# seqsense/pcgol

Hardware: AMD Instinct MI355X
Metric: Mpoints/sec ICP iter (corr+reduce) + kNN queries/sec, 1M-pt cloud (higher is better)
Workload: dtype f32

## Files before the change

pcgol_amd/csrc/icp.hip:

```cpp
#include <string.h>

#include <array>
#include <chrono>
#include <condition_variable>
#include <mutex>
#include <string>
#include <thread>

#include <vector>

#include "knn_grid.h"
#include "knn_xwalk.h"
#include "strict_terms.h"

namespace pcgx {

constexpr int kIcpBlock = kKnnBlock;

__device__ __forceinline__ double wave_sum_f64(double v) {
#pragma unroll
  for (int o = 32; o > 0; o >>= 1) v += __shfl_down(v, o);
  return v;
}

// ... 145 lines not shown
      return;
    }
  }
  uint32_t *queue = s_stack + (size_t)(tv.depth > 1 ? tv.depth - 1 : 1) * kIcpBlock +
                    (threadIdx.x >> 6) * (kWalkQueueBytesPerWave / 4);
  float *top = reinterpret_cast<float *>(s_stack + (size_t)(tv.depth > 1 ? tv.depth - 1 : 1) * kIcpBlock +
                                         (kIcpBlock / 64) * (kWalkQueueBytesPerWave / 4));
  load_top_levels(tv, top);
  uint32_t chunk_begin, chunk_end;
  block_chunk_range(nt, blockIdx.x, gridDim.x, chunk_begin, chunk_end);
  if (threadIdx.x == 0) s_next_chunk = chunk_begin;
  __syncthreads();
  float m[16];
#pragma unroll
  for (int i = 0; i < 16; i++) m[i] = state->trans[i];
  const bool project = state->iter > 0;
  auto load_query = [&](int64_t i, float &x, float &y, float &z, float &ub, uint32_t &pred) {
    const float x0 = tx[i], y0 = ty[i], z0 = tz[i];
    float4 pm = make_float4(0.0f, 0.0f, 0.0f, -1.0f);
    pred = 0u;
    if (project) {
      pred = first_leaf[i] & 0x7fffffffu;
      if (!kMinDist) pm = match[i];
    }
    x = x0; y = y0; z = z0;
    if (project) mat4_transform(m, x0, y0, z0, x, y, z);
    const float dx = pm.x - x, dy = pm.y - y, dz = pm.z - z;
    const float dm = (dx * dx + dy * dy) + dz * dz;
    ub = dm + (pm.w >= 0.0f ? 0.0f : __builtin_inff());
  };
  auto emit = [&](int64_t i, const float4 &bp, float best_d) {
    const float4 rec = make_float4(bp.x, bp.y, bp.z, __float_as_int(bp.w) >= 0 ? best_d : -1.0f);
    match[i] = rec;
    if (match_caller) match_caller[orig_of[i]] = rec;
    if (kPlane) match_id[i] = __float_as_uint(bp.w);
    if (match_cert) match_cert[i] = (cert_by_id && __float_as_int(bp.w) >= 0) ? cert_by_id[__float_as_uint(bp.w)] : 0.0f;
  };
  if (kGrid) {
    const int64_t r_begin = (int64_t)chunk_begin * 64;
    __syncthreads();
    if (threadIdx.x == 0) {
      walk_count[slot] = 0;
      s_next_chunk = 0;
    }
    __syncthreads();
    walk_queries<kMinDist>(
        tv, s_stack + threadIdx.x, kIcpBlock, queue, top, (int64_t)left, &s_next_chunk, (left + 63u) / 64u, 0,
        kp.max_dist_sq, kp.min_dist_sq,
        [&](int64_t j, float &x, float &y, float &z, float &ub, uint32_t &pred) {
          load_query(r_begin + walk_list[r_begin + j], x, y, z, ub, pred);
          pred &= 0x7fffffffu;
        },
        [&](int64_t j, const float4 &bp, float best_d) { emit(r_begin + walk_list[r_begin + j], bp, best_d); },
        [&](int64_t j, uint32_t leaf) { first_leaf[r_begin + walk_list[r_begin + j]] = kSums ? (leaf | 0x80000000u) : leaf; });
    if (!kSums) {
      __syncthreads();
      strict_tile_sums();
      return;
    }
    __threadfence_block();
    __syncthreads();
    reduce_block_range<kPlane, true>(s_stack, tx, ty, tz, nt, chunk_begin, chunk_end, project, m, match, match_id,
                                     normals, kp, block_partials, first_leaf, grid_part);
    return;
  } else {
    walk_queries<kMinDist>(
        tv, s_stack + threadIdx.x, kIcpBlock, queue, top, nt, &s_next_chunk, chunk_end, (int64_t)chunk_begin * 64,
// ... 58 lines not shown
      if (test_force_walk && i % test_force_walk == 0) kept = false;
      if (kTrace && match_cert != nullptr && grid.cert != nullptr && pm.w >= 0.0f && dm < match_cert[i] && dm < kp.max_dist_sq)
        atomicAdd(&trace[36], 1ull);
    }
    float4 best = make_float4(0.0f, 0.0f, 0.0f, __int_as_float(-1));
    float best_d = kp.max_dist_sq;
    GridTrace tr;
    GridVerdict v = GRID_FOUND;
    if (kept) {
      best = make_float4(pm.x, pm.y, pm.z, __int_as_float(0));
      best_d = dm;
    } else {
      v = grid_nearest(grid, x, y, z, kp.max_dist_sq, ub, best, best_d, kTrace ? &tr : nullptr);
      if (test_force_walk && project && i % test_force_walk == 0) v = GRID_WALK;
    }
    if (use_cert && !kept)
      match_cert[i] = (v == GRID_FOUND && __float_as_int(best.w) >= 0) ? grid.cert[__float_as_uint(best.w)] : 0.0f;
    if (kTrace) {
      if (v == GRID_WALK) atomicAdd(&trace[0], 1ull);
      atomicAdd(&trace[1], (unsigned long long)tr.points);
      atomicAdd(&trace[2], (unsigned long long)tr.words);
      if (tr.wave_slots) atomicAdd(&trace[3], (unsigned long long)tr.wave_slots);
      atomicAdd(&trace[4 + (tr.rounds4 < 0 ? 0 : min(tr.rounds4 + 1, 15))], 1ull);
      atomicAdd(&trace[20 + (tr.rounds9 < 0 ? 0 : min(tr.rounds9 + 1, 15))], 1ull);
    } else if (v == GRID_WALK) {
      uint32_t begin;
      const uint32_t slot = slot_of_query(nt, i, n_corr_blocks, begin);
      const int64_t r_begin = (int64_t)begin * 64;
      walk_list[r_begin + atomicAdd(&walk_count[slot], 1u)] = (uint32_t)(i - r_begin);
      first_leaf[i] = kSums ? 0x80000000u : 0u;
      if (!walk_follows) const_cast<IcpState *>(state)->done = 2;
      if (!kSums && match_caller) {
        const bool seen = __float_as_int(best.w) >= 0;
        match_caller[orig_of[i]] = make_float4(best.x, best.y, best.z, seen ? best_d : -1.0f);
      }
    } else {
      const bool found = __float_as_int(best.w) >= 0;
      const float4 bp = make_float4(best.x, best.y, best.z, found ? best_d : -1.0f);
      if (kept) reinterpret_cast<float *>(&match[i])[3] = bp.w;
      else match[i] = bp;
      if (!kSums && match_caller && !(kept && caller_has_pairs)) match_caller[orig_of[i]] = bp;
      if (kPlane && !kept) match_id[i] = __float_as_uint(best.w);
      if (found && kSums) {
        if (kPlane) accumulate_plane_terms(acc, x, y, z, bp, normals[kept ? match_id[i] : __float_as_uint(best.w)]);
        else accumulate_terms(acc, x, y, z, bp, kp);
      }
    }
  }
  if (kTrace || !kSums) return;
  constexpr int kSub = kPlane ? 8 : 16, kRun = kIcpGridBlock / kSub;
  static_assert(NS * kSub <= kIcpGridBlock, "one lane per (component, run)");
#pragma unroll
  for (int k = 0; k < NS; k++) s_terms[k][threadIdx.x] = (float)acc[k];
  __syncthreads();
  if (threadIdx.x < NS * kSub) {
    const int k = threadIdx.x / kSub, j = threadIdx.x % kSub;
    double v = 0.0;
    for (int u = 0; u < kRun; u++) v += (double)s_terms[k][u * kSub + j];
#pragma unroll
    for (int o = kSub / 2; o > 0; o >>= 1) v += __shfl_down(v, o, kSub);
    if (j == 0) block_partials[((int64_t)n_corr_blocks + tile) * NS + k] = v;
  }
}

template <bool kMinDist, bool kPlane, bool kSums = true>
__global__ __launch_bounds__(kIcpBlock) void icp_corr_xkernel(
    XTreeView xv, const float *__restrict__ tx, const float *__restrict__ ty, const float *__restrict__ tz,
    int64_t nt, const IcpState *__restrict__ state, IcpKernelParams kp, float4 *__restrict__ match,
    double *__restrict__ block_partials, uint32_t *__restrict__ match_id, const float4 *__restrict__ normals,
    int64_t guard) {
  extern __shared__ uint32_t s_stack[];
  if (state->done) return;
  uint32_t chunk_begin, chunk_end;
  block_chunk_range(nt, blockIdx.x, gridDim.x, chunk_begin, chunk_end);
// ... 152 lines not shown

using namespace pcgx;

struct pcgx_icp_session {
  const pcgx_kdtree *base = nullptr;
  bool patched = false;
  int64_t nt = 0;
  float *d_xyz = nullptr;
  IcpState *d_state = nullptr;
  double *d_partials = nullptr;
  uint32_t *d_pos_of = nullptr;
  uint32_t *d_orig_of = nullptr;
  float4 *d_match_caller = nullptr;
  bool caller_order_fresh = false;
  bool tile_sums_fresh = false;
  int strict = 0;
  bool strict_explicit = false;
  pcgx::StrictBuffers *strict_buf = nullptr;
  float *d_terms = nullptr;
  unsigned long long *d_valid = nullptr;
  int64_t nt_pad = 0;
  float4 *d_match = nullptr;
  float *d_match_cert = nullptr;
  uint32_t *d_first_leaf = nullptr;
  uint32_t *d_walk_list = nullptr;
  uint32_t *d_walk_count = nullptr;
  double *d_sums = nullptr;
  bool own_sums = false;
  double *d_xchg = nullptr;
  int32_t steps_sharded = 0;
  int32_t host_iter = 0;
  bool spec_walk = true;
  bool spec_pending = false;
  hipStream_t spec_stream = nullptr;
  hipStream_t used[4] = {nullptr, nullptr, nullptr, nullptr};
  int n_used = 0;
  void touch(hipStream_t st) {
    for (int k = 0; k < n_used && k < 4; k++)
      if (used[k] == st) return;
    if (n_used > 0) (void)hipStreamSynchronize(used[0]);
    if (n_used < 4) used[n_used] = st;
    n_used++;
  }
  bool shard_failed = false;
  bool ring_fit_open = false;
  bool general_ready = true;
  bool small = false;
  int32_t *d_small_perm = nullptr;
  void *d_small_sync = nullptr;
  bool plane = false;
  uint32_t *d_match_id = nullptr;
  float4 *d_normals = nullptr;
  int n_sums() const { return plane ? (int)P_COUNT : (int)S_COUNT; }
  int grid = 1;
  IcpKernelParams kp;
  int32_t max_iteration = 20;
};

static pcgx_status settle(pcgx_icp_session *s, hipStream_t st);
static int icp_knob(const char *name, int def, int lo, int hi);

static IcpKernelParams make_kernel_params(const pcgx_icp_params *p) {
  IcpKernelParams kp;
  memset(&kp, 0, sizeof kp);
  kp.max_dist_sq = p->max_dist * p->max_dist;
  kp.min_dist_sq = p->min_dist_sq;
// ... 11 lines not shown
  if (blocks > cap) blocks = cap;
  if (blocks >= 8) blocks &= ~(int64_t)7;
  if (blocks < 1) blocks = 1;
  return (int)blocks;
}

__global__ void icp_reset_kernel(IcpState *__restrict__ state) {
  if (threadIdx.x != 0 || blockIdx.x != 0) return;
  IcpState h;
  memset(&h, 0, sizeof h);
  const Mat4 id = mat4_translate(0.0f, 0.0f, 0.0f);
  for (int i = 0; i < 16; i++) h.trans[i] = id.m[i];
  *state = h;
}

static pcgx_status general_prepare(pcgx_icp_session *s, hipStream_t st) {
  if (s->general_ready) return PCGX_OK;
  const size_t n1 = (size_t)(s->nt ? s->nt : 1);
  PCGX_HIP_TRY(hipMemsetAsync(s->d_match, 0xFF, n1 * sizeof(float4), st));
  PCGX_HIP_TRY(hipMemsetAsync(s->d_match_cert, 0, n1 * sizeof(float), st));
  PCGX_HIP_TRY(hipMemsetAsync(s->d_first_leaf, 0, n1 * sizeof(uint32_t), st));
  PCGX_HIP_TRY(hipMemsetAsync(s->d_walk_count, 0, (size_t)s->grid * sizeof(uint32_t), st));
  s->general_ready = true;
  return PCGX_OK;
}

static pcgx_status reset_state(pcgx_icp_session *s, hipStream_t st) {
  hipLaunchKernelGGL(icp_reset_kernel, dim3(1), dim3(64), 0, st, s->d_state);
  PCGX_HIP_TRY(hipGetLastError());
  s->host_iter = 0;
  if (s->spec_pending) {
    s->spec_pending = false;
    if (s->d_walk_count) PCGX_HIP_TRY(hipMemsetAsync(s->d_walk_count, 0, (size_t)s->grid * sizeof(uint32_t), st));
  }
  if (s->shard_failed || s->steps_sharded > 0) {
    PCGX_TRY(strict_reset(s->strict_buf, st));
    s->shard_failed = false;
    s->steps_sharded = 0;
  }
  return PCGX_OK;
}

extern "C" pcgx_status pcgx_icp_session_reset(pcgx_icp_session *s, void *stream) {
  PCGX_API_LOCK();
  if (!s) return fail(PCGX_E_INVALID, "pcgx_icp_session_reset: NULL session");
  s->touch(pick_stream(stream));
  return reset_state(s, pick_stream(stream));
}

extern "C" pcgx_status pcgx_icp_session_set_pose(pcgx_icp_session *s, const float trans16[16],
                                                 int32_t iter, void *stream) {
  PCGX_API_LOCK();
  if (!s || !trans16 || iter < 0) return fail(PCGX_E_INVALID, "pcgx_icp_session_set_pose: bad argument");
  hipStream_t st = pick_stream(stream);
  s->touch(st);
  PCGX_TRY(settle(s, st));
  IcpState h;
  memset(&h, 0, sizeof h);
  memcpy(h.trans, trans16, sizeof h.trans);
  h.iter = iter;
  s->host_iter = 0;
  PCGX_HIP_TRY(hipMemcpyAsync(s->d_state, &h, sizeof h, hipMemcpyHostToDevice, st));
  PCGX_HIP_TRY(hipStreamSynchronize(st));
  return PCGX_OK;
}

// ... 244 lines not shown
  }
  return def;
}

static pcgx_status enqueue_corr_patched(pcgx_icp_session *s, hipStream_t st) {
  XTreeView xv;
  PCGX_TRY(xtree_view(s->base, &xv, st));
  const size_t lds = (size_t)(xv.depth > 1 ? xv.depth : 2) * kIcpBlock * sizeof(uint32_t);
  const int64_t guard = 4 * s->base->n + 8;
  const float *x = s->d_xyz, *y = s->d_xyz + s->nt, *z = s->d_xyz + 2 * s->nt;
  ProfScope prof(PCGX_PROF_ICP_WALK, st);
  if (s->plane)
    hipLaunchKernelGGL((icp_corr_xkernel<false, true>), dim3(s->grid), dim3(kIcpBlock), lds, st, xv, x, y, z, s->nt,
                       s->d_state, s->kp, s->d_match, s->d_partials, s->d_match_id, (const float4 *)s->d_normals, guard);
  else if (s->kp.min_dist_sq > 0.0f && s->strict)
    hipLaunchKernelGGL((icp_corr_xkernel<true, false, false>), dim3(s->grid), dim3(kIcpBlock), lds, st, xv, x, y, z, s->nt,
                       s->d_state, s->kp, s->d_match, s->d_partials, (uint32_t *)nullptr, (const float4 *)nullptr, guard);
  else if (s->kp.min_dist_sq > 0.0f)
    hipLaunchKernelGGL((icp_corr_xkernel<true, false>), dim3(s->grid), dim3(kIcpBlock), lds, st, xv, x, y, z, s->nt,
                       s->d_state, s->kp, s->d_match, s->d_partials, (uint32_t *)nullptr, (const float4 *)nullptr, guard);
  else if (s->strict)
    hipLaunchKernelGGL((icp_corr_xkernel<false, false, false>), dim3(s->grid), dim3(kIcpBlock), lds, st, xv, x, y, z, s->nt,
                       s->d_state, s->kp, s->d_match, s->d_partials, (uint32_t *)nullptr, (const float4 *)nullptr, guard);
  else
    hipLaunchKernelGGL((icp_corr_xkernel<false, false>), dim3(s->grid), dim3(kIcpBlock), lds, st, xv, x, y, z, s->nt,
                       s->d_state, s->kp, s->d_match, s->d_partials, (uint32_t *)nullptr, (const float4 *)nullptr, guard);
  PCGX_HIP_TRY(hipGetLastError());
  return PCGX_OK;
}

static pcgx_status enqueue_corr(pcgx_icp_session *s, hipStream_t st, bool may_speculate = false) {
  static const int tight = icp_knob("PCGX_ICP_TIGHT", 32, 0, 32), chunks = icp_knob("PCGX_ICP_CHUNKS", 2, 1, 64);
  if (!s->patched && s->base->n_deleted > 0) s->patched = true;
  PCGX_TRY(general_prepare(s, st));
  const bool caller_had_pairs = s->caller_order_fresh;
  s->caller_order_fresh = false;
  s->tile_sums_fresh = false;
  if (s->patched) return enqueue_corr_patched(s, st);
  if (s->strict == 1 && !s->plane && s->nt > 0) {
    if (!s->d_match_caller) {
      hipError_t e = dev_cache_alloc((void **)&s->d_orig_of, (size_t)s->nt * sizeof(uint32_t));
      if (e == hipSuccess) e = dev_cache_alloc((void **)&s->d_match_caller, (size_t)s->nt * sizeof(float4));
      if (e != hipSuccess) {
        (void)hipGetLastError();
        dev_cache_free(s->d_orig_of);
        dev_cache_free(s->d_match_caller);
        s->d_orig_of = nullptr;
        s->d_match_caller = nullptr;
      } else {
        hipLaunchKernelGGL(invert_positions_kernel, dim3((unsigned)((s->nt + 255) / 256)), dim3(256), 0, st,
                           (const uint32_t *)s->d_pos_of, s->nt, s->d_orig_of);
      }
    }
    s->caller_order_fresh = s->d_match_caller != nullptr;
    if (!s->strict_buf)
      PCGX_TRY(strict_create(s->nt, s->d_xyz, s->d_xyz + s->nt, s->d_xyz + 2 * s->nt, (const uint32_t *)s->d_pos_of,
                             &s->strict_buf, st));
  }
  TreeView tv = s->base->view();
  tv.tight_levels = tight;
  tv.chunks_per_refill = chunks;
  const size_t lds = walk_lds_bytes(tv, kIcpBlock);
  const float *x = s->d_xyz, *y = s->d_xyz + s->nt, *z = s->d_xyz + 2 * s->nt;
  const bool grid = grid_enabled(s->base) && !(s->kp.min_dist_sq > 0.0f) && s->nt > 0;
  s->tile_sums_fresh = grid && s->caller_order_fresh && s->strict == 1 && !s->plane && !strict_work(s->strict_buf, s->kp)->exchange;
  const StrictWork strict_w = s->tile_sums_fresh ? *strict_work(s->strict_buf, s->kp) : StrictWork();
  static const int left_blocks = icp_knob("PCGX_ICP_LEFTOVER_BLOCKS", 128, 8, 4096) & ~7;
  const int n_corr = (grid && s->strict && !s->plane && s->grid > left_blocks) ? left_blocks : s->grid;
  static const bool cert_on = icp_knob("PCGX_ICP_CERT", 1, 0, 1) != 0;
  float *cert = (grid && cert_on && s->base->grid.cert) ? s->d_match_cert : nullptr;
  static const bool spec_on = icp_knob("PCGX_ICP_SPEC_WALK", 1, 0, 1) != 0;
  static const int test_force_walk = icp_knob("PCGX_TEST_ICP_FORCE_WALK", 0, 0, 1 << 30);
  const bool no_walk = may_speculate && spec_on && s->spec_walk && grid && s->strict == 1 && !s->plane && s->host_iter >= 1 &&
                       !s->tile_sums_fresh;
  if (no_walk) {
    s->spec_pending = true;
    s->spec_stream = st;
  }
  if (grid) {
    ProfScope prof_grid(PCGX_PROF_ICP_GRID, st);
    const unsigned gb = (unsigned)((s->nt + kIcpGridBlock - 1) / kIcpGridBlock);
    if (s->plane)
      hipLaunchKernelGGL(icp_grid_kernel<true>, dim3(xcd_grid(gb)), dim3(kIcpGridBlock), 0, st, s->base->grid, x, y, z, s->nt,
                         s->d_state, s->kp, s->d_match, s->d_match_id, (const float4 *)s->d_normals, s->d_first_leaf,
                         s->d_walk_list, s->d_walk_count, (uint32_t)s->grid, s->d_partials, (unsigned long long *)nullptr,
                         (const uint32_t *)nullptr, (float4 *)nullptr, cert);
    else if (s->strict)
      hipLaunchKernelGGL((icp_grid_kernel<false, false, false>),
                         dim3(xcd_grid((unsigned)((s->nt + kIcpStrictGridBlock - 1) / kIcpStrictGridBlock))),
                         dim3(kIcpStrictGridBlock), 0, st, s->base->grid, x, y, z,
                         s->nt, s->d_state, s->kp, s->d_match, s->d_match_id, (const float4 *)s->d_normals,
                         s->d_first_leaf, s->d_walk_list, s->d_walk_count, (uint32_t)n_corr, s->d_partials,
                         (unsigned long long *)nullptr, (const uint32_t *)(s->caller_order_fresh ? s->d_orig_of : nullptr),
                         s->caller_order_fresh ? s->d_match_caller : nullptr, cert, caller_had_pairs ? 1 : 0, no_walk ? 0 : 1, test_force_walk);
    else
      hipLaunchKernelGGL(icp_grid_kernel<false>, dim3(xcd_grid(gb)), dim3(kIcpGridBlock), 0, st, s->base->grid, x, y, z, s->nt,
                         s->d_state, s->kp, s->d_match, s->d_match_id, (const float4 *)s->d_normals, s->d_first_leaf,
                         s->d_walk_list, s->d_walk_count, (uint32_t)s->grid, s->d_partials, (unsigned long long *)nullptr,
                         (const uint32_t *)nullptr, (float4 *)nullptr, cert);
  }
  if (no_walk) return PCGX_OK;
  ProfScope prof(grid ? PCGX_PROF_ICP_LEFTOVER : PCGX_PROF_ICP_WALK, st);
#define PCGX_LAUNCH_CORR(MD, PL, GR)                                                                                  \
  do {                                                                                                                \
  if (s->strict && !PL)                                                                                               \
    hipLaunchKernelGGL((icp_corr_kernel<MD, false, GR, false>), dim3(n_corr), dim3(kIcpBlock), lds, st, tv, x, y, z, \
                       s->nt, s->d_state, s->kp, s->d_match, s->d_first_leaf, s->d_partials, s->d_match_id,           \
                       (const float4 *)s->d_normals, s->d_walk_list, s->d_walk_count,                                 \
                       (int32_t)((s->nt + kIcpGridBlock - 1) / kIcpGridBlock),                                        \
                       (const uint32_t *)(s->caller_order_fresh ? s->d_orig_of : nullptr),                            \
                       s->caller_order_fresh ? s->d_match_caller : nullptr, strict_w,                                 \
                       (int32_t)((GR) && s->tile_sums_fresh ? 1 : 0), cert, s->base->grid.cert);                      \
  else                                                                                                                \
  hipLaunchKernelGGL((icp_corr_kernel<MD, PL, GR>), dim3(s->grid), dim3(kIcpBlock), lds, st, tv, x, y, z, s->nt,     \
                     s->d_state, s->kp, s->d_match, s->d_first_leaf, s->d_partials, s->d_match_id,                   \
                     (const float4 *)s->d_normals, s->d_walk_list, s->d_walk_count,                                  \
                     (int32_t)((s->nt + kIcpGridBlock - 1) / kIcpGridBlock), (const uint32_t *)nullptr,               \
                     (float4 *)nullptr, StrictWork(), 0, cert, s->base->grid.cert);                                   \
  } while (0)
  if (s->plane) {
    if (grid) PCGX_LAUNCH_CORR(false, true, true);
    else PCGX_LAUNCH_CORR(false, true, false);
  } else if (s->kp.min_dist_sq > 0.0f) {
    PCGX_LAUNCH_CORR(true, false, false);
  } else {
    if (grid) PCGX_LAUNCH_CORR(false, false, true);
    else PCGX_LAUNCH_CORR(false, false, false);
  }
#undef PCGX_LAUNCH_CORR
  return PCGX_OK;
}

template <bool kFuseUpdate>
static pcgx_status enqueue_strict(pcgx_icp_session *s, hipStream_t st) {
  if (s->strict == 1) {
    if (!s->strict_buf)
      PCGX_TRY(strict_create(s->nt, s->d_xyz, s->d_xyz + s->nt, s->d_xyz + 2 * s->nt, (const uint32_t *)s->d_pos_of,
                             &s->strict_buf, st));
    const bool first_iter = s->host_iter++ == 0;
    if (s->caller_order_fresh)
      PCGX_TRY(strict_enqueue(s->strict_buf, (const float4 *)s->d_match_caller, (const uint32_t *)nullptr, s->d_state,
                              s->d_sums, s->kp, kFuseUpdate, s->tile_sums_fresh, first_iter, st));
    else
      PCGX_TRY(strict_enqueue(s->strict_buf, (const float4 *)s->d_match, (const uint32_t *)s->d_pos_of, s->d_state,
                              s->d_sums, s->kp, kFuseUpdate, false, first_iter, st));
    return PCGX_OK;
  }
  if (!s->d_terms) {
    s->nt_pad = (s->nt + 63) & ~(int64_t)63;
    const size_t np = (size_t)(s->nt_pad ? s->nt_pad : 64);
    PCGX_HIP_TRY(dev_cache_alloc((void **)&s->d_terms, 9 * np * sizeof(float)));
    PCGX_HIP_TRY(dev_cache_alloc((void **)&s->d_valid, (np / 64) * sizeof(unsigned long long)));
  }
  return strict_check_enqueue(s->d_xyz, s->nt, s->nt_pad, (const float4 *)s->d_match, (const uint32_t *)s->d_pos_of, s->d_state, s->kp,
                              s->d_terms, s->d_valid, s->d_sums, kFuseUpdate, st);
}

static pcgx_status settle(pcgx_icp_session *s, hipStream_t st) {
  if (!s->spec_pending) return PCGX_OK;
  s->spec_pending = false;
  IcpState h;
  PCGX_HIP_TRY(hipMemcpyAsync(&h, s->d_state, sizeof h, hipMemcpyDeviceToHost, st));
  PCGX_HIP_TRY(hipStreamSynchronize(st));
  if (h.done != 2) return PCGX_OK;
  s->spec_walk = false;
  const int32_t missing = s->host_iter - h.num_iteration;
  if (getenv("PCGX_ICP_SPEC_TRACE"))
    fprintf(stderr, "pcgx icp: a step without the leftover walk met a target the grid could not answer: %d of %d Evaluates enqueued again, with the walk\n",
            (int)missing, (int)s->host_iter);
  const int32_t zero = 0;
  PCGX_HIP_TRY(hipMemcpyAsync(&s->d_state->done, &zero, sizeof zero, hipMemcpyHostToDevice, st));
  PCGX_HIP_TRY(hipMemsetAsync(s->d_walk_count, 0, (size_t)s->grid * sizeof(uint32_t), st));
  s->host_iter = h.num_iteration;
  for (int32_t k = 0; k < missing; k++) {
    PCGX_TRY(enqueue_corr(s, st, false));
    PCGX_TRY(enqueue_strict<true>(s, st));
  }
  PCGX_HIP_TRY(hipGetLastError());
  return PCGX_OK;
}

extern "C" pcgx_status pcgx_debug_icp_strict_stats(pcgx_icp_session *s, void *stream, int64_t out[64]) {
  PCGX_API_LOCK();
  if (!s || !out) return fail(PCGX_E_INVALID, "pcgx_debug_icp_strict_stats: NULL argument");
  for (int k = 0; k < 64; k++) out[k] = 0;
  if (!s->strict_buf) return PCGX_OK;
  PCGX_TRY(settle(s, pick_stream(stream)));
  unsigned long long h[64];
  PCGX_TRY(strict_read_debug(s->strict_buf, h, pick_stream(stream)));
  for (int k = 0; k < 64; k++) out[k] = (int64_t)h[k];
  return PCGX_OK;
}

extern "C" pcgx_status pcgx_icp_session_partials(pcgx_icp_session *s, void *stream) {
  PCGX_API_LOCK();
  if (!s) return fail(PCGX_E_INVALID, "pcgx_icp_session_partials: NULL session");
  hipStream_t st = pick_stream(stream);
  s->touch(st);
  PCGX_TRY(settle(s, st));
  PCGX_TRY(enqueue_corr(s, st));
  if (s->strict)
    PCGX_TRY(enqueue_strict<false>(s, st));
  else if (s->plane)
    hipLaunchKernelGGL((icp_final_reduce_kernel<false, true>), dim3(1), dim3(1024), 0, st, s->d_partials, s->grid,
                       s->d_state, s->d_sums, s->kp);
// ... 536 lines not shown
```

pcgol_amd/csrc/pcgx_internal.h:

```cpp
#pragma once
#include <hip/hip_runtime.h>
#include <stdint.h>
#include <stdio.h>
#include <stdlib.h>

#include <atomic>
#include <memory>
#include <mutex>
#include <string>
#include <utility>
#include <vector>

#include "../../include/pcgx.h"
#include "pcgx_math.h"

namespace pcgx {

template <class T>
struct DefaultInitAlloc : std::allocator<T> {
  template <class U>
  struct rebind {
    using other = DefaultInitAlloc<U>;
  };
  template <class U>
// ... 249 lines not shown
  PCGX_DPP_ADD(0x114, 0xf);
  PCGX_DPP_ADD(0x118, 0xf);
  PCGX_DPP_ADD(0x142, 0xa);
  PCGX_DPP_ADD(0x143, 0xc);
#undef PCGX_DPP_ADD
  return v;
}
__device__ __forceinline__ void icp_update_step(IcpState *__restrict__ state, const double *__restrict__ sums10,
                                                const IcpKernelParams &kp) {
  state->num_iteration += 1;
  const int64_t npairs = (int64_t)sums10[S_PAIRS];
  if (npairs < (int64_t)kp.min_pairs) {
    state->ev.num_pairs = npairs;
    state->status = PCGX_E_NOT_ENOUGH_PAIRS;
    state->done = 1;
    return;
  }
  Evaluated ev;
  finish_evaluate(sums10, ev);
  state->ev = ev;
  Mat4 t;
  for (int i = 0; i < 16; i++) t.m[i] = state->trans[i];
  int32_t it = state->iter;
  const bool converged = gradient_descent_update(kp.upd, it, ev.gradient, t);
  for (int i = 0; i < 16; i++) state->trans[i] = t.m[i];
  state->iter = it;
  if (converged) state->done = 1;
}

#endif

struct StrictBuffers;
struct StrictWork;
pcgx_status strict_create(int64_t nt, const float *tx, const float *ty, const float *tz, const uint32_t *pos_of,
                          StrictBuffers **out, hipStream_t st);
void strict_destroy(StrictBuffers *b);
const StrictWork *strict_work(StrictBuffers *b, const IcpKernelParams &kp);
pcgx_status strict_enqueue(StrictBuffers *b, const float4 *match, const uint32_t *pos_of, IcpState *state,
                           double *sums10, const IcpKernelParams &kp, bool fuse_update, bool have_tile_sums, bool first_iter,
                           hipStream_t st);
pcgx_status strict_read_debug(StrictBuffers *b, unsigned long long out[64], hipStream_t st);
pcgx_status strict_check_enqueue(const float *d_xyz, int64_t nt, int64_t nt_pad, const float4 *match, const uint32_t *pos_of,
                                 IcpState *state, const IcpKernelParams &kp, float *d_terms, unsigned long long *d_valid,
                                 double *d_sums, bool fuse_update, hipStream_t st);
pcgx_status strict_enqueue_sharded(StrictBuffers *b, const float4 *match, const uint32_t *pos_of, IcpState *state,
                                   double *sums10, const IcpKernelParams &kp, pcgx_comm *c, int rank, int world,
                                   bool local_failed, hipStream_t st);
struct RingView {
  unsigned long long *words = nullptr;
  unsigned long long *host = nullptr;
  unsigned long long *const *tab = nullptr;
  unsigned long long *mine = nullptr;
  int32_t words_per_rank = 0, rank = 0, world = 1;
  uint32_t epoch = 0;
  int32_t kind = 0;
  long long guess_ticks = 0;
};
pcgx_status strict_enqueue_ring(StrictBuffers *b, const float4 *match, const uint32_t *pos_of, IcpState *state, double *sums10,
                                const IcpKernelParams &kp, const RingView &ring, bool local_failed, bool first_iter, hipStream_t st);
void ring_abort_from_host(const RingView &ring, uint32_t reason);
pcgx_status strict_reset(StrictBuffers *b, hipStream_t st);
bool small_fit_eligible(const TreeView &tv, int64_t nt, bool many_ties);
size_t small_fit_sync_bytes();
size_t small_fit_terms_bytes(int64_t nt);
int small_fit_max_iters();
bool small_fit_wants_order(int64_t nt);
pcgx_status small_fit_prepare(const float *d_target_aos, int64_t nt, const float box_lo[3], const float box_hi[3], int32_t *d_perm, float *d_xyz,
                               uint32_t *d_pos_of, IcpState *state, void *terms, void *sync, hipStream_t st);
pcgx_status small_fit_enqueue(const TreeView &tv, const float *tx, const float *ty, const float *tz, int64_t nt, IcpState *state,
                              const IcpKernelParams &kp, void *terms, unsigned long long *valid, double *sums10, void *sync,
                              uint32_t launch_no, int iters, const int32_t *perm, hipStream_t st, volatile uint32_t *mailbox = nullptr,
                              uint32_t mailbox_seq = 0u);
bool comm_ring_step(pcgx_comm *c, int32_t step, RingView *out);
// ... 56 lines not shown
```

pcgol_amd/csrc/strict.hip:

```cpp
#include <stddef.h>

#include "strict_terms.h"

namespace pcgx {

__device__ __forceinline__ int lane_next(int v, int edge) { return __builtin_amdgcn_update_dpp(edge, v, 0x130, 0xf, 0xf, false); }
__device__ __forceinline__ int lane_prev(int v, int edge) { return __builtin_amdgcn_update_dpp(edge, v, 0x138, 0xf, 0xf, false); }
__device__ __forceinline__ double wave_excl_scan_f64(double v, int lane) {
  double inc = v;
  inc += dpp_f64<0x111, 0xf>(0.0, inc);
  inc += dpp_f64<0x112, 0xf>(0.0, inc);
  inc += dpp_f64<0x114, 0xf>(0.0, inc);
  inc += dpp_f64<0x118, 0xf>(0.0, inc);
  inc += dpp_f64<0x142, 0xa>(0.0, inc);
  inc += dpp_f64<0x143, 0xc>(0.0, inc);
  (void)lane;
  return dpp_f64<0x138, 0xf>(0.0, inc);
}
__device__ __forceinline__ uint32_t wave_all_umin(uint32_t v) {
#define PCGX_DPP_U32(CTRL, MASK) (uint32_t) __builtin_amdgcn_update_dpp(-1, (int)v, CTRL, MASK, 0xf, false)
  v = umin(v, PCGX_DPP_U32(0x111, 0xf));
  v = umin(v, PCGX_DPP_U32(0x112, 0xf));
  v = umin(v, PCGX_DPP_U32(0x114, 0xf));
  v = umin(v, PCGX_DPP_U32(0x118, 0xf));
  v = umin(v, PCGX_DPP_U32(0x142, 0xa));
  v = umin(v, PCGX_DPP_U32(0x143, 0xc));
#undef PCGX_DPP_U32
  return (uint32_t)__builtin_amdgcn_readlane((int)v, 63);
}
__device__ __forceinline__ uint32_t wave_all_umax(uint32_t v) {
#define PCGX_DPP_U32(CTRL, MASK) (uint32_t) __builtin_amdgcn_update_dpp(0, (int)v, CTRL, MASK, 0xf, false)
  v = umax(v, PCGX_DPP_U32(0x111, 0xf));
  v = umax(v, PCGX_DPP_U32(0x112, 0xf));
  v = umax(v, PCGX_DPP_U32(0x114, 0xf));
// ... 249 lines not shown
                                             ChainRange &cr, double &tile_err) {
  g = f2u((float)(base + pre));
  const float e = u2f(plain_chain_q(q, g));
  const double err = ((double)e - (double)u2f(g)) - lsum;
  const double epre = wave_excl_scan_f64(err, lane);
  tile_err = lane_f64(epre, 63) + lane_f64(err, 63);
  const uint32_t g2 = f2u((float)(base + pre + epre));
  const int32_t moved = (int32_t)g2 - (int32_t)g;
  if (__ballot(moved > 2 || moved < -2) != 0ull) g = g2;
  cr = guess_chain_q(q, g);
}
__device__ __forceinline__ void tile_guesses_pair(const LdsQuads &q, double base, double lsum, double pre, int lane, uint32_t &g,
                                                  ChainRange &cr, ChainRange &crb, double &tile_err) {
  g = f2u((float)(base + pre));
  const float e = u2f(plain_chain_q(q, g));
  const double err = ((double)e - (double)u2f(g)) - lsum;
  const double epre = wave_excl_scan_f64(err, lane);
  tile_err = lane_f64(epre, 63) + lane_f64(err, 63);
  const uint32_t g2 = f2u((float)(base + pre + epre));
  const int32_t moved = (int32_t)g2 - (int32_t)g;
  if (__ballot(moved > 2 || moved < -2) != 0ull) g = g2;
  guess_chain_pair_q(q, g, cr, crb);
}

constexpr int kExactTiles = 1;
constexpr uint32_t kPlainMargin = 512u;
constexpr uint32_t kMaybeMargin = 1u << 17;

constexpr int kSumBlock = 512;
constexpr int kSumWaves = kSumBlock / 64;
enum { JOB_CROSSING = 1, JOB_NOWINDOW = 2 };

constexpr long long kExchangeTicks = 200000;
template <bool kExchange, bool kSharded = false>
__global__ __launch_bounds__(kSumBlock) __attribute__((amdgpu_waves_per_eu(4, 4))) void strict_sum_kernel(
    const float4 *__restrict__ match, const uint32_t *__restrict__ pos_of, const IcpState *__restrict__ state, StrictWork W) {
  __shared__ float4 s_terms[kStrictRows][kTile / 4];
  __shared__ int s_np[kSumWaves];
  __shared__ double s_tot[16];
  static_assert(!kSharded || kExchange, "the ring form rides on the exchange");
  const int done = state->done;
  const int lane = threadIdx.x & 63, wave = threadIdx.x >> 6;
  const int64_t tile = blockIdx.x;
  const int NR = W.nrows;
  const long long t_0 = trace_clock(W);
  long long t_x0 = 0;
  double P0 = (!kExchange && wave < NR) ? tile_prefix(W.tile_sum, W.ntiles, wave, tile, lane) : 0.0;
  {
    const TermSrc S = make_term_src(match, pos_of, state, W);
    const int l = threadIdx.x >> 3, v = threadIdx.x & 7;
    float4 bp[4];
    float tx[4], ty[4], tz[4];
    load_quad(S, tile * kTile + (int64_t)l * kLeaf + 4 * v, bp, tx, ty, tz);
    float t[4][kStrictRows];
    int np = 0;
#pragma unroll
    for (int c = 0; c < 4; c++) np += pair_terms(S, tx[c], ty[c], tz[c], bp[c], t[c]) ? 1 : 0;
#pragma unroll
    for (int k = 0; k < kStrictRows; k++) s_terms[k][tile_quad(l, v)] = make_float4(t[0][k], t[1][k], t[2][k], t[3][k]);
#pragma unroll
    for (int o = 32; o > 0; o >>= 1) np += __shfl_xor(np, o);
    if (lane == 0) s_np[wave] = np;
  }
  __syncthreads();
  if (done) return;
  if (threadIdx.x == 0) {
    int np = 0;
    for (int w = 0; w < kSumWaves; w++) np += s_np[w];
    W.tile_pairs[tile] = (uint32_t)np;
  }
  static_assert(kStrictRows <= 2 * kSumWaves, "a wave has at most two rows");
  double lsum_kept[2] = {0.0, 0.0}, pre_kept[2] = {0.0, 0.0};
  if (kExchange) {
#pragma unroll
    for (int pass = 0; pass < 2; pass++) {
      const int row = wave + pass * kSumWaves;
      if (row >= NR) break;
      const LdsQuads q{s_terms[row], lane};
      double lsum = 0.0;
#pragma unroll
      for (int v = 0; v < kLeaf / 4; v++) {
        const float4 a = q(v);
        lsum += (double)a.x; lsum += (double)a.y; lsum += (double)a.z; lsum += (double)a.w;
      }
      const double pre = wave_excl_scan_f64(lsum, lane);
      lsum_kept[pass] = lsum;
      pre_kept[pass] = pre;
      if (lane == 63) s_tot[row] = pre + lsum;
    }
    __syncthreads();
    t_x0 = trace_clock(W);
    if (wave == 0) {
      if (lane < NR) {
        const double v = s_tot[lane];
        __hip_atomic_store(&W.tile_pub[(int64_t)lane * W.ntiles_pad + tile], v, __ATOMIC_RELAXED, __HIP_MEMORY_SCOPE_AGENT);
        W.tile_sum[(int64_t)lane * W.ntiles + tile] = v;
      }
      asm volatile("s_waitcnt vmcnt(0)" ::: "memory");
      const int64_t g_mine = tile >> 5, n_groups = (W.ntiles + 31) >> 5;
      if (lane == 0) {
// ... 1806 lines not shown

const StrictWork *strict_work(StrictBuffers *b, const IcpKernelParams &kp) {
  b->w.weight_fn = kp.weight_fn;
  b->w.weight_a = kp.weight_a;
  b->w.nrows = kp.weight_fn == PCGX_WEIGHT_ONE ? kStrictRows - 1 : kStrictRows;
  return &b->w;
}
static bool repair_enabled() {
  static const bool on = !(getenv("PCGX_STRICT_REPAIR") && atoi(getenv("PCGX_STRICT_REPAIR")) == 0);
  return on;
}
static const StrictWork &next_epoch(StrictBuffers *b) {
  if (++b->w.epoch == 0u) b->w.epoch = 1u;
  return b->w;
}

static bool spec_enabled() {
  static const bool on = !(getenv("PCGX_STRICT_SPEC") && atoi(getenv("PCGX_STRICT_SPEC")) == 0);
  return on;
}
static void launch_chain(const StrictWork &W, const float4 *match, const uint32_t *pos_of, IcpState *state, double *sums10,
                         const IcpKernelParams &kp, int fuse_update, bool waits, hipStream_t st) {
  const dim3 grid((unsigned)(W.nrows * W.nchunks)), block(kChainBlock);
  if (W.selfcheck & 1)
    hipLaunchKernelGGL((strict_chain_kernel<true, false>), grid, block, 0, st, match, pos_of, state, W, sums10, kp, fuse_update);
  else if (waits && spec_enabled() && (W.ring ? W.rank : 0) * W.nchunks + W.nchunks - 1 >= W.spec_depth)
    hipLaunchKernelGGL((strict_chain_kernel<false, true>), grid, block, 0, st, match, pos_of, state, W, sums10, kp, fuse_update);
  else
    hipLaunchKernelGGL((strict_chain_kernel<false, false>), grid, block, 0, st, match, pos_of, state, W, sums10, kp, fuse_update);
}

pcgx_status strict_enqueue(StrictBuffers *b, const float4 *match, const uint32_t *pos_of, IcpState *state,
                           double *sums10, const IcpKernelParams &kp, bool fuse_update, bool have_tile_sums, bool first_iter,
                           hipStream_t st) {
  (void)strict_work(b, kp);
  const StrictWork &W = next_epoch(b);
  if (!have_tile_sums && !W.exchange) {
    ProfScope prof(PCGX_PROF_STRICT_TERMS, st);
    hipLaunchKernelGGL(strict_tilesum_kernel, dim3((unsigned)W.ntiles), dim3(kTileSumBlock), 0, st, match, pos_of,
                       (const IcpState *)state, W);
  }
  {
    ProfScope prof(PCGX_PROF_STRICT_SUM, st);
    if (W.exchange)
      hipLaunchKernelGGL(strict_sum_kernel<true>, dim3((unsigned)W.ntiles), dim3(kSumBlock), 0, st, match, pos_of,
                         (const IcpState *)state, W);
    else
      hipLaunchKernelGGL(strict_sum_kernel<false>, dim3((unsigned)W.ntiles), dim3(kSumBlock), 0, st, match, pos_of,
                         (const IcpState *)state, W);
  }
  {
    ProfScope prof(PCGX_PROF_STRICT_JOB, st);
    if (first_iter && W.naux > 0 && W.ntiles >= kRepairMinTiles && repair_enabled())
      hipLaunchKernelGGL(strict_repair_kernel, dim3((unsigned)(W.nrows * ((W.ntiles + kRepairBlock - 1) / kRepairBlock))), dim3(kRepairBlock), 0,
                         st, match, pos_of, (const IcpState *)state, W);
    if (W.naux > 0)
      hipLaunchKernelGGL(strict_job_kernel, dim3((unsigned)kJobRoles * (unsigned)W.naux), dim3(kJobBlock), 0, st, (const IcpState *)state, W);
  }
  {
    ProfScope prof(PCGX_PROF_STRICT_CHAIN, st);
    launch_chain(W, match, pos_of, state, sums10, kp, fuse_update ? 1 : 0, W.nchunks > 1, st);
  }
  PCGX_HIP_TRY(hipGetLastError());
  return PCGX_OK;
}

__global__ __launch_bounds__(64) void strict_row_totals_kernel(const double *__restrict__ per_tile, const uint32_t *__restrict__ tile_pairs,
                                                               int64_t ntiles, int nrows, const IcpState *__restrict__ state,
                                                               double *__restrict__ slot ) {
  const int row = blockIdx.x, lane = threadIdx.x;
  if (state->done) return;
  if (row < nrows) {
    double v = 0.0;
    for (int64_t t = lane; t < ntiles; t += 64) v += per_tile[(int64_t)row * ntiles + t];
    v = wave_allsum_f64(v);
    if (lane == 0) slot[row] = v;
  } else if (row == kStrictRows && tile_pairs) {
// ... 317 lines not shown
```

pcgol_amd/csrc/strict_terms.h:

```cpp
#pragma once
#include "pcgx_internal.h"
#include "strict_sum.h"

namespace pcgx {
using namespace ss;

constexpr int kStrictRows = 9;


template <int kCtrl, int kRowMask>
__device__ __forceinline__ double dpp_f64(double old, double v) {
  constexpr bool kZeroFill = kRowMask == 0xf;
  const unsigned long long o = (unsigned long long)__double_as_longlong(old), x = (unsigned long long)__double_as_longlong(v);
  const uint32_t lo = (uint32_t)__builtin_amdgcn_update_dpp((int)(uint32_t)o, (int)(uint32_t)x, kCtrl, kRowMask, 0xf, kZeroFill);
  const uint32_t hi = (uint32_t)__builtin_amdgcn_update_dpp((int)(uint32_t)(o >> 32), (int)(uint32_t)(x >> 32), kCtrl, kRowMask, 0xf, kZeroFill);
  return __longlong_as_double((long long)((unsigned long long)hi << 32 | lo));
}
__device__ __forceinline__ double lane_f64(double v, int src) {
  const unsigned long long x = (unsigned long long)__double_as_longlong(v);
  const uint32_t lo = (uint32_t)__builtin_amdgcn_readlane((int)(uint32_t)x, src), hi = (uint32_t)__builtin_amdgcn_readlane((int)(uint32_t)(x >> 32), src);
  return __longlong_as_double((long long)((unsigned long long)hi << 32 | lo));
}
__device__ __forceinline__ double wave_allsum_f64(double v) {
  v += dpp_f64<0x111, 0xf>(0.0, v);
// ... 48 lines not shown
  uint32_t *cand;
  unsigned int *aux_count;
  unsigned int *done_rows;
  unsigned long long *dbg;
  unsigned long long *stamps;
  int64_t nt, ntiles;
  int32_t naux;
  int32_t nrows;
  int32_t weight_fn;
  float weight_a;
  const float *raw_terms;
  int32_t exchange;
  const double *row_base;
  const double *err_base;
  const uint32_t *start_bits;
  double *hop_out;
  int32_t first_exact;
  unsigned long long *chunk_state;
  int32_t nchunks;
  uint32_t epoch;
  unsigned long long *ring;
  int32_t ring_words;
  unsigned long long *const *ring_tab;
  unsigned long long *ring_mine;
  int32_t rank, world;
  uint32_t ring_epoch;
  long long ring_guess_ticks;
  double *ring_base;
  unsigned int *ring_flag;
  int32_t spec_depth;
  int32_t selfcheck;
};

struct RingLayout {
  int world;
  __host__ __device__ int row_tot(int k, int row) const { return (k * kStrictRows + row) * 2; }
  __host__ __device__ int err_tot(int k, int row) const { return world * 2 * kStrictRows + (k * kStrictRows + row) * 2; }
  __host__ __device__ int start(int row) const { return world * 4 * kStrictRows + row; }
  __host__ __device__ int start_pairs() const { return world * 4 * kStrictRows + kStrictRows; }
  __host__ __device__ int final(int row) const { return world * 4 * kStrictRows + 16 + row; }
  __host__ __device__ int final_pairs() const { return world * 4 * kStrictRows + 16 + kStrictRows; }
  __host__ __device__ int abort() const { return world * 4 * kStrictRows + 32; }
  __host__ __device__ int words() const { return (world * 4 * kStrictRows + 33 + 15) & ~15; }
};
constexpr int kRingTagStepBits = 12;
constexpr long long kRingGuessTicks = 200000;
constexpr long long kRingGuessTicksApart = 20000000;
constexpr long long kRingWalkTicks = 1000000000;

#if defined(__HIPCC__)
__device__ __forceinline__ void ring_put(unsigned long long *w, uint32_t payload, uint32_t epoch) {
  __hip_atomic_store(w, (unsigned long long)epoch << 32 | payload, __ATOMIC_RELAXED, __HIP_MEMORY_SCOPE_SYSTEM);
}
__device__ __forceinline__ void ring_put_f64(unsigned long long *w, double v, uint32_t epoch) {
  const unsigned long long x = (unsigned long long)__double_as_longlong(v);
  ring_put(w, (uint32_t)x, epoch);
  ring_put(w + 1, (uint32_t)(x >> 32), epoch);
}
__device__ __forceinline__ bool ring_peek(const unsigned long long *w, uint32_t epoch, uint32_t &payload) {
  const unsigned long long v = __hip_atomic_load(w, __ATOMIC_RELAXED, __HIP_MEMORY_SCOPE_SYSTEM);
  payload = (uint32_t)v;
  return (uint32_t)(v >> 32) == epoch;
}
__device__ __forceinline__ bool ring_aborted(const StrictWork &W) {
  const RingLayout RL{W.world};
  const unsigned long long v = __hip_atomic_load(W.ring + (size_t)W.rank * W.ring_words + RL.abort(), __ATOMIC_RELAXED, __HIP_MEMORY_SCOPE_SYSTEM);
// ... 168 lines not shown
```

Before: 14040.

## Fuse correspondence search into strict-sum kernel for late ICP iterations

From the second host iteration onward, when the caller-order pairs are fresh and the exchange path is active, the separate correspondence kernel is skipped. The strict sum kernel instead checks each point's previous match for validity and reruns the grid nearest search only for points that fail, writing terms into shared memory. The match_caller w-field now carries the certificate value instead of the distance, and extra strict_reset calls are added on reset paths. This removes one full pass over the cloud and a kernel launch per iteration, at the cost of more complex sum-kernel code, higher LDS use and possible divergence from the in-kernel search.

```diff
diff --git a/pcgol_amd/csrc/icp.hip b/pcgol_amd/csrc/icp.hip
--- a/pcgol_amd/csrc/icp.hip
+++ b/pcgol_amd/csrc/icp.hip
@@ -201,7 +201,9 @@
   auto emit = [&](int64_t i, const float4 &bp, float best_d) {
     const float4 rec = make_float4(bp.x, bp.y, bp.z, __float_as_int(bp.w) >= 0 ? best_d : -1.0f);
     match[i] = rec;
-    if (match_caller) match_caller[orig_of[i]] = rec;
+    if (match_caller)
+      match_caller[orig_of[i]] = make_float4(rec.x, rec.y, rec.z,
+                                             rec.w >= 0.0f ? (cert_by_id ? cert_by_id[__float_as_uint(bp.w)] : 0.0f) : -1.0f);
     if (kPlane) match_id[i] = __float_as_uint(bp.w);
     if (match_cert) match_cert[i] = (cert_by_id && __float_as_int(bp.w) >= 0) ? cert_by_id[__float_as_uint(bp.w)] : 0.0f;
   };
@@ -326,14 +328,17 @@
       if (!walk_follows) const_cast<IcpState *>(state)->done = 2;
       if (!kSums && match_caller) {
         const bool seen = __float_as_int(best.w) >= 0;
-        match_caller[orig_of[i]] = make_float4(best.x, best.y, best.z, seen ? best_d : -1.0f);
+        match_caller[orig_of[i]] = make_float4(best.x, best.y, best.z, seen ? 0.0f : -1.0f);
       }
     } else {
       const bool found = __float_as_int(best.w) >= 0;
       const float4 bp = make_float4(best.x, best.y, best.z, found ? best_d : -1.0f);
       if (kept) reinterpret_cast<float *>(&match[i])[3] = bp.w;
       else match[i] = bp;
-      if (!kSums && match_caller && !(kept && caller_has_pairs)) match_caller[orig_of[i]] = bp;
+      if (!kSums && match_caller && !(kept && caller_has_pairs)) {
+        const float c = kept ? pm_cert : ((use_cert && v == GRID_FOUND && found) ? grid.cert[__float_as_uint(best.w)] : 0.0f);
+        match_caller[orig_of[i]] = make_float4(bp.x, bp.y, bp.z, found ? c : -1.0f);
+      }
       if (kPlane && !kept) match_id[i] = __float_as_uint(best.w);
       if (found && kSums) {
         if (kPlane) accumulate_plane_terms(acc, x, y, z, bp, normals[kept ? match_id[i] : __float_as_uint(best.w)]);
@@ -552,6 +557,7 @@
   int32_t host_iter = 0;
   bool spec_walk = true;
   bool spec_pending = false;
+  bool certify_next = false;
   hipStream_t spec_stream = nullptr;
   hipStream_t used[4] = {nullptr, nullptr, nullptr, nullptr};
   int n_used = 0;
@@ -629,6 +635,7 @@
   if (s->spec_pending) {
     s->spec_pending = false;
     if (s->d_walk_count) PCGX_HIP_TRY(hipMemsetAsync(s->d_walk_count, 0, (size_t)s->grid * sizeof(uint32_t), st));
+    PCGX_TRY(strict_reset(s->strict_buf, st));
   }
   if (s->shard_failed || s->steps_sharded > 0) {
     PCGX_TRY(strict_reset(s->strict_buf, st));
@@ -939,6 +946,7 @@
 static pcgx_status enqueue_corr(pcgx_icp_session *s, hipStream_t st, bool may_speculate = false) {
   static const int tight = icp_knob("PCGX_ICP_TIGHT", 32, 0, 32), chunks = icp_knob("PCGX_ICP_CHUNKS", 2, 1, 64);
   if (!s->patched && s->base->n_deleted > 0) s->patched = true;
+  s->certify_next = false;
   PCGX_TRY(general_prepare(s, st));
   const bool caller_had_pairs = s->caller_order_fresh;
   s->caller_order_fresh = false;
@@ -984,6 +992,10 @@
     s->spec_pending = true;
     s->spec_stream = st;
   }
+  static const int fused_from = icp_knob("PCGX_ICP_FUSED_FROM", 2, 0, 1 << 30);
+  s->certify_next = no_walk && fused_from > 0 && s->host_iter >= fused_from && cert != nullptr && caller_had_pairs &&
+                    s->caller_order_fresh && strict_work(s->strict_buf, s->kp)->exchange;
+  if (s->certify_next) return PCGX_OK;
   if (grid) {
     ProfScope prof_grid(PCGX_PROF_ICP_GRID, st);
     const unsigned gb = (unsigned)((s->nt + kIcpGridBlock - 1) / kIcpGridBlock);
@@ -1045,7 +1057,22 @@
       PCGX_TRY(strict_create(s->nt, s->d_xyz, s->d_xyz + s->nt, s->d_xyz + 2 * s->nt, (const uint32_t *)s->d_pos_of,
                              &s->strict_buf, st));
     const bool first_iter = s->host_iter++ == 0;
-    if (s->caller_order_fresh)
+    if (s->certify_next) {
+      s->certify_next = false;
+      static const int force_search = icp_knob("PCGX_TEST_ICP_FUSED_SEARCH", 0, 0, 1 << 30);
+      static const int force_grid_walk = icp_knob("PCGX_TEST_ICP_FUSED_GRID_WALK", 0, 0, 1 << 30);
+      CertifiedTerms C;
+      C.grid = s->base->grid;
+      C.max_dist_sq = s->kp.max_dist_sq;
+      C.match_caller = s->d_match_caller;
+      C.match = s->d_match;
+      C.match_cert = s->d_match_cert;
+      C.pos_of = s->d_pos_of;
+      C.test_force_walk = force_search;
+      C.test_force_grid_walk = force_grid_walk;
+      PCGX_TRY(strict_enqueue(s->strict_buf, (const float4 *)s->d_match_caller, (const uint32_t *)nullptr, s->d_state,
+                              s->d_sums, s->kp, kFuseUpdate, false, first_iter, st, &C));
+    } else if (s->caller_order_fresh)
       PCGX_TRY(strict_enqueue(s->strict_buf, (const float4 *)s->d_match_caller, (const uint32_t *)nullptr, s->d_state,
                               s->d_sums, s->kp, kFuseUpdate, s->tile_sums_fresh, first_iter, st));
     else
@@ -1078,6 +1105,7 @@
   const int32_t zero = 0;
   PCGX_HIP_TRY(hipMemcpyAsync(&s->d_state->done, &zero, sizeof zero, hipMemcpyHostToDevice, st));
   PCGX_HIP_TRY(hipMemsetAsync(s->d_walk_count, 0, (size_t)s->grid * sizeof(uint32_t), st));
+  PCGX_TRY(strict_reset(s->strict_buf, st));
   s->host_iter = h.num_iteration;
   for (int32_t k = 0; k < missing; k++) {
     PCGX_TRY(enqueue_corr(s, st, false));
diff --git a/pcgol_amd/csrc/pcgx_internal.h b/pcgol_amd/csrc/pcgx_internal.h
--- a/pcgol_amd/csrc/pcgx_internal.h
+++ b/pcgol_amd/csrc/pcgx_internal.h
@@ -305,13 +305,14 @@
 
 struct StrictBuffers;
 struct StrictWork;
+struct CertifiedTerms;
 pcgx_status strict_create(int64_t nt, const float *tx, const float *ty, const float *tz, const uint32_t *pos_of,
                           StrictBuffers **out, hipStream_t st);
 void strict_destroy(StrictBuffers *b);
 const StrictWork *strict_work(StrictBuffers *b, const IcpKernelParams &kp);
 pcgx_status strict_enqueue(StrictBuffers *b, const float4 *match, const uint32_t *pos_of, IcpState *state,
                            double *sums10, const IcpKernelParams &kp, bool fuse_update, bool have_tile_sums, bool first_iter,
-                           hipStream_t st);
+                           hipStream_t st, const struct CertifiedTerms *certify = nullptr);
 pcgx_status strict_read_debug(StrictBuffers *b, unsigned long long out[64], hipStream_t st);
 pcgx_status strict_check_enqueue(const float *d_xyz, int64_t nt, int64_t nt_pad, const float4 *match, const uint32_t *pos_of,
                                  IcpState *state, const IcpKernelParams &kp, float *d_terms, unsigned long long *d_valid,
diff --git a/pcgol_amd/csrc/strict.hip b/pcgol_amd/csrc/strict.hip
--- a/pcgol_amd/csrc/strict.hip
+++ b/pcgol_amd/csrc/strict.hip
@@ -1,5 +1,6 @@
 #include <stddef.h>
 
+#include "knn_grid.h"
 #include "strict_terms.h"
 
 namespace pcgx {
@@ -315,13 +316,61 @@
 enum { JOB_CROSSING = 1, JOB_NOWINDOW = 2 };
 
 constexpr long long kExchangeTicks = 200000;
-template <bool kExchange, bool kSharded = false>
+__device__ __forceinline__ void certified_search(const CertifiedTerms &C, const TermSrc &S, const IcpState *state, const StrictWork &W,
+                                                 int64_t tile, const uint16_t *list, int nl, float4 *terms ,
+                                                 int *np_more) {
+  TermSrc S0 = S;
+  S0.project = false;
+  for (int j = threadIdx.x; j < nl; j += kSumBlock) {
+    const int q = list[j];
+    const int64_t c = tile * kTile + q;
+    float x = W.xyz_caller[3 * c], y = W.xyz_caller[3 * c + 1], z = W.xyz_caller[3 * c + 2];
+    float ub = __builtin_inff();
+    if (S.project) {
+      float px, py, pz;
+      mat4_transform(S.m, x, y, z, px, py, pz);
+      x = px; y = py; z = pz;
+      const float4 pm = C.match_caller[c];
+      const float dx = pm.x - x, dy = pm.y - y, dz = pm.z - z;
+      const float dm = (dx * dx + dy * dy) + dz * dz;
+      if (pm.w >= 0.0f && dm == dm) ub = dm;
+    }
+    float4 best = make_float4(0.0f, 0.0f, 0.0f, __int_as_float(-1));
+    float best_d = C.max_dist_sq;
+    GridVerdict v = grid_nearest(C.grid, x, y, z, C.max_dist_sq, ub, best, best_d);
+    if (C.test_force_grid_walk && c % C.test_force_grid_walk == 0) v = GRID_WALK;
+    if (v == GRID_WALK) {
+      if (atomicCAS(&const_cast<IcpState *>(state)->done, 0, 2) == 0) atomicAdd(&W.dbg[47], 1ull << 32);
+      continue;
+    }
+    const bool found = __float_as_int(best.w) >= 0;
+    const float cert = (v == GRID_FOUND && found) ? C.grid.cert[__float_as_uint(best.w)] : 0.0f;
+    const uint32_t pos = C.pos_of[c];
+    C.match[pos] = make_float4(best.x, best.y, best.z, found ? best_d : -1.0f);
+    C.match_cert[pos] = cert;
+    C.match_caller[c] = make_float4(best.x, best.y, best.z, found ? cert : -1.0f);
+    if (found) {
+      float t[kStrictRows];
+      (void)pair_terms(S0, x, y, z, make_float4(best.x, best.y, best.z, best_d), t);
+      const int l = q / kLeaf, vq = (q % kLeaf) / 4, cc = q % 4;
+#pragma unroll
+      for (int k = 0; k < kStrictRows; k++) reinterpret_cast<float *>(&terms[k * (kTile / 4) + tile_quad(l, vq)])[cc] = t[k];
+      atomicAdd(np_more, 1);
+    }
+  }
+}
+
+template <bool kExchange, bool kSharded = false, bool kCertify = false>
 __global__ __launch_bounds__(kSumBlock) __attribute__((amdgpu_waves_per_eu(4, 4))) void strict_sum_kernel(
-    const float4 *__restrict__ match, const uint32_t *__restrict__ pos_of, const IcpState *__restrict__ state, StrictWork W) {
+    const float4 *__restrict__ match, const uint32_t *__restrict__ pos_of, const IcpState *__restrict__ state, StrictWork W,
+    CertifiedTerms C = CertifiedTerms()) {
   __shared__ float4 s_terms[kStrictRows][kTile / 4];
   __shared__ int s_np[kSumWaves];
   __shared__ double s_tot[16];
+  __shared__ uint16_t s_list[kCertify ? kTile : 1];
+  __shared__ int s_nlist, s_np_more;
   static_assert(!kSharded || kExchange, "the ring form rides on the exchange");
+  static_assert(!kCertify || (kExchange && !kSharded), "the certified terms: one GPU, with the exchange");
   const int done = state->done;
   const int lane = threadIdx.x & 63, wave = threadIdx.x >> 6;
   const int64_t tile = blockIdx.x;
@@ -334,11 +383,31 @@
     const int l = threadIdx.x >> 3, v = threadIdx.x & 7;
     float4 bp[4];
     float tx[4], ty[4], tz[4];
-    load_quad(S, tile * kTile + (int64_t)l * kLeaf + 4 * v, bp, tx, ty, tz);
+    const int64_t i0 = tile * kTile + (int64_t)l * kLeaf + 4 * v;
+    load_quad(S, i0, bp, tx, ty, tz);
+    if (kCertify) {
+      if (threadIdx.x == 0) s_nlist = s_np_more = 0;
+      __syncthreads();
+    }
     float t[4][kStrictRows];
     int np = 0;
 #pragma unroll
-    for (int c = 0; c < 4; c++) np += pair_terms(S, tx[c], ty[c], tz[c], bp[c], t[c]) ? 1 : 0;
+    for (int c = 0; c < 4; c++) {
+      if (kCertify) {
+        float x = tx[c], y = ty[c], z = tz[c];
+        if (S.project) mat4_transform(S.m, tx[c], ty[c], tz[c], x, y, z);
+        const float dx = bp[c].x - x, dy = bp[c].y - y, dz = bp[c].z - z;
+        const float dm = (dx * dx + dy * dy) + dz * dz;
+        bool kept = S.project && bp[c].w >= 0.0f && dm < bp[c].w && dm < C.max_dist_sq;
+        if ((C.test_force_walk && (i0 + c) % C.test_force_walk == 0) || (C.test_force_grid_walk && (i0 + c) % C.test_force_grid_walk == 0))
+          kept = false;
+        if (!kept && i0 + c < W.nt) {
+          s_list[atomicAdd(&s_nlist, 1)] = (uint16_t)(l * kLeaf + 4 * v + c);
+          bp[c].w = -1.0f;
+        }
+      }
+      np += pair_terms(S, tx[c], ty[c], tz[c], bp[c], t[c]) ? 1 : 0;
+    }
 #pragma unroll
     for (int k = 0; k < kStrictRows; k++) s_terms[k][tile_quad(l, v)] = make_float4(t[0][k], t[1][k], t[2][k], t[3][k]);
 #pragma unroll
@@ -347,8 +416,19 @@
   }
   __syncthreads();
   if (done) return;
+  if (kCertify) {
+    const int nl = s_nlist;
+    if (nl > 0) {
+      certified_search(C, make_term_src(match, pos_of, state, W), state, W, tile, s_list, nl, &s_terms[0][0], &s_np_more);
+      __syncthreads();
+    }
+    if (threadIdx.x == 0) {
+      if (tile == 0) atomicAdd(&W.dbg[47], 1ull);
+      if (nl > 0) atomicAdd(&W.dbg[59], (unsigned long long)nl);
+    }
+  }
   if (threadIdx.x == 0) {
-    int np = 0;
+    int np = kCertify ? s_np_more : 0;
     for (int w = 0; w < kSumWaves; w++) np += s_np[w];
     W.tile_pairs[tile] = (uint32_t)np;
   }
@@ -2221,7 +2301,7 @@
 
 pcgx_status strict_enqueue(StrictBuffers *b, const float4 *match, const uint32_t *pos_of, IcpState *state,
                            double *sums10, const IcpKernelParams &kp, bool fuse_update, bool have_tile_sums, bool first_iter,
-                           hipStream_t st) {
+                           hipStream_t st, const CertifiedTerms *certify) {
   (void)strict_work(b, kp);
   const StrictWork &W = next_epoch(b);
   if (!have_tile_sums && !W.exchange) {
@@ -2231,7 +2311,12 @@
   }
   {
     ProfScope prof(PCGX_PROF_STRICT_SUM, st);
-    if (W.exchange)
+    if (certify && W.exchange && !pos_of)
+      hipLaunchKernelGGL((strict_sum_kernel<true, false, true>), dim3((unsigned)W.ntiles), dim3(kSumBlock), 0, st, match,
+                         pos_of, (const IcpState *)state, W, *certify);
+    else if (certify)
+      return fail(PCGX_E_INVALID, "strict sums: the certified terms need the exchange and the pairs in the caller's order");
+    else if (W.exchange)
       hipLaunchKernelGGL(strict_sum_kernel<true>, dim3((unsigned)W.ntiles), dim3(kSumBlock), 0, st, match, pos_of,
                          (const IcpState *)state, W);
     else
diff --git a/pcgol_amd/csrc/strict_terms.h b/pcgol_amd/csrc/strict_terms.h
--- a/pcgol_amd/csrc/strict_terms.h
+++ b/pcgol_amd/csrc/strict_terms.h
@@ -104,6 +104,17 @@
   int32_t selfcheck;
 };
 
+struct CertifiedTerms {
+  GridView grid;
+  float max_dist_sq;
+  float4 *match_caller;
+  float4 *match;
+  float *match_cert;
+  const uint32_t *pos_of;
+  int32_t test_force_walk;
+  int32_t test_force_grid_walk;
+};
+
 struct RingLayout {
   int world;
   __host__ __device__ int row_tot(int k, int row) const { return (k * kStrictRows + row) * 2; }
```

After: 14870, median of 6. +5.9%, better.
